# AlessioSam/LADiff

Measured on AMD Instinct MI355X. Metric: motions/sec (196-frame, 50-step DDIM, bs128), higher is better.
Workload: dtype f16x3+f32; 1 GPU; headline:ddim50_cfg7.5_b128_f196_c263_humanml3d; prompts_per_gpu=128, global_batch=128, frames=196, scheduler=ddim, denoising_steps=50, parallelism=dp1, loop=persistent pipeline kernel (16-row blocks x 86)

## Files before the change

include/ladiff_hip_debug.h:

```cpp
#ifndef LADIFF_HIP_DEBUG_H
#define LADIFF_HIP_DEBUG_H

#include "ladiff_hip.h"

#ifdef __cplusplus
extern "C" {
#endif

LADIFF_API int ladiff_debug_set_stage_waves(int waves_per_simd);
LADIFF_API int ladiff_debug_set_handoff(int tagged);
LADIFF_API int ladiff_debug_set_stage_plan(int v);
LADIFF_API int ladiff_debug_set_poll_pause(int mask, int len);
LADIFF_API int ladiff_debug_set_stage_delay(int mask, int len);
LADIFF_API int ladiff_debug_set_pacing(int eighths, int mask);
LADIFF_API int ladiff_debug_set_xcd_local(int on);
LADIFF_API int ladiff_debug_set_decoder_fusion(int on);
LADIFF_API int ladiff_debug_set_mlp_variant(int v);

LADIFF_API int ladiff_debug_set_loop_thresholds(int look_ahead_from, int small_upto);
LADIFF_API int ladiff_debug_set_graph_epoch_rule(int on);
LADIFF_API int ladiff_debug_graph_instantiations(void);

#ifdef LADIFF_STAMPS
LADIFF_API void ladiff_debug_set_stamps(unsigned long long* p);
LADIFF_API void ladiff_debug_set_sys_stamps(unsigned long long* p);
LADIFF_API void ladiff_debug_set_probe(int v);
#endif

#ifdef __cplusplus
}
#endif
#endif
```

ladiff_amd/_lib.py:

```python
import ctypes
import os
from ctypes import c_char_p, c_float, c_int, c_size_t, c_uint64, c_void_p

import numpy as np
import torch

_HERE = os.path.dirname(os.path.abspath(__file__))
LIB_PATH = os.path.join(_HERE, "libladiff_hip.so")

MAX_LATENTS = 8
MAX_FRAMES = 224
COEF_STRIDE = 8
ACT = {"none": 0, "relu": 1, "gelu": 2, "silu": 3, "qgelu": 4, "lrelu": 5}


class LadiffHipError(RuntimeError):
    pass


SPLIT_MODES = ("f16x3", "bf16x3", "split")


def is_split(precision):
    if precision == "fp32":
# ... 61 lines not shown
    "ladiff_debug_set_stage_plan": (c_int, [c_int]),
    "ladiff_debug_set_poll_pause": (c_int, [c_int, c_int]),
    "ladiff_debug_set_stage_delay": (c_int, [c_int, c_int]),
    "ladiff_debug_set_pacing": (c_int, [c_int, c_int]),
    "ladiff_debug_set_loop_thresholds": (c_int, [c_int, c_int]),
    "ladiff_debug_set_graph_epoch_rule": (c_int, [c_int]),
    "ladiff_debug_graph_instantiations": (c_int, []),
    "ladiff_sampler_set_fault": (c_int, [c_void_p, c_int, c_int]),
    "ladiff_sampler_set_noise_generator": (c_int, [c_void_p, c_uint64, ctypes.c_uint32, c_int]),
    "ladiff_noise_fill": (c_int, [c_uint64, ctypes.c_uint32, c_int, c_int, c_int, c_int, c_void_p, c_void_p]),
    "ladiff_reverse_workspace_bytes": (c_size_t, [c_int, c_int, c_int, c_int]),
    "ladiff_diffusion_reverse": (c_int, [c_void_p, c_void_p, c_void_p, c_uint64, c_void_p, c_void_p, c_void_p, c_void_p, c_void_p,
                                         c_void_p, c_void_p, c_void_p, c_float, c_float, c_int, c_int, c_int, c_int, c_int,
                                         c_void_p, c_void_p, c_size_t, c_int, c_void_p]),
    "ladiff_encoder_num_params": (c_int, []),
    "ladiff_encoder_param_name": (c_char_p, [c_int]),
    "ladiff_encoder_workspace_bytes": (c_size_t, [c_int, c_int, c_int, c_int]),
    "ladiff_vae_encode": (c_int, [c_void_p, c_void_p, c_void_p, c_void_p, c_void_p, c_void_p, c_int, c_int, c_int, c_int,
                                  c_void_p, c_void_p, c_void_p, c_void_p, c_size_t, c_void_p]),
    "ladiff_clip_num_params": (c_int, []),
    "ladiff_clip_param_name": (c_char_p, [c_int]),
    "ladiff_clip_workspace_bytes": (c_size_t, [c_int, c_int]),
    "ladiff_clip_text_encode": (c_int, [c_void_p, c_void_p, c_int, c_int, c_void_p, c_int, c_int, c_int, c_void_p, c_void_p,
                                        c_size_t, c_void_p]),
    "ladiff_clip_workspace_bytes_ragged": (c_size_t, [c_int, c_int]),
    "ladiff_clip_text_encode_ragged": (c_int, [c_void_p, c_void_p, c_int, c_int, c_void_p, c_int, c_int, c_int, c_void_p, c_void_p,
                                               c_void_p, c_int, c_void_p, c_void_p, c_size_t, c_void_p]),
    "ladiff_t2m_movement_num_params": (c_int, []),
    "ladiff_t2m_movement_param_name": (c_char_p, [c_int]),
    "ladiff_t2m_motion_num_params": (c_int, []),
    "ladiff_t2m_motion_param_name": (c_char_p, [c_int]),
    "ladiff_t2m_text_num_params": (c_int, []),
    "ladiff_t2m_text_param_name": (c_char_p, [c_int]),
    "ladiff_t2m_movement_workspace_bytes": (c_size_t, [c_int, c_int, c_int]),
    "ladiff_t2m_motion_workspace_bytes": (c_size_t, [c_int, c_int]),
    "ladiff_t2m_text_workspace_bytes": (c_size_t, [c_int, c_int]),
    "ladiff_t2m_movement_encode": (c_int, [c_void_p, c_void_p, c_int, c_int, c_int, c_int, c_void_p, c_void_p, c_size_t,
                                           c_void_p]),
    "ladiff_t2m_motion_encode": (c_int, [c_void_p, c_void_p, c_void_p, c_int, c_int, c_void_p, c_void_p, c_size_t, c_void_p]),
    "ladiff_t2m_text_encode": (c_int, [c_void_p, c_void_p, c_void_p, c_void_p, c_int, c_int, c_void_p, c_void_p, c_size_t,
                                       c_void_p]),
    "ladiff_feats2joints": (c_int, [c_void_p, c_void_p, c_void_p, c_int, c_int, c_int, c_int, c_void_p, c_void_p]),
    "ladiff_joint_ape_ave": (c_int, [c_void_p, c_void_p, c_void_p, c_void_p, c_int, c_int, c_int, c_void_p, c_float, c_void_p, c_void_p,
                                     c_void_p]),
    "ladiff_joint_mr": (c_int, [c_void_p, c_void_p, c_void_p, c_int, c_int, c_int, c_void_p, c_void_p, c_void_p]),
    "ladiff_decoder_workspace_bytes": (c_size_t, [c_int, c_int, c_int, c_int]),
    "ladiff_vae_decode": (c_int, [c_void_p, c_void_p, c_void_p, c_void_p, c_void_p, c_int, c_int, c_int, c_int, c_void_p,
                                  c_void_p, c_size_t, c_void_p]),
    "ladiff_debug_set_stage_waves": (c_int, [c_int]),
    "ladiff_debug_set_handoff": (c_int, [c_int]),
    "ladiff_debug_set_xcd_local": (c_int, [c_int]),
    "ladiff_debug_set_decoder_fusion": (c_int, [c_int]),
    "ladiff_debug_set_mlp_variant": (c_int, [c_int]),
    "ladiff_reverse_plan": (c_int, [c_int, c_int, c_void_p, c_int, c_int, c_int, c_int, c_void_p, c_void_p]),
    "ladiff_decoder_graph_create": (c_int, [ctypes.POINTER(c_void_p)]),
    "ladiff_decoder_graph_destroy": (c_int, [c_void_p]),
    "ladiff_vae_decode_graphed": (c_int, [c_void_p, c_void_p, c_void_p, c_uint64, c_void_p, c_void_p, c_void_p, c_void_p, c_int, c_int, c_int,
                                          c_int, c_int, c_void_p, c_void_p, c_size_t, c_void_p]),
    "ladiff_vae_decode_ragged": (c_int, [c_void_p, c_void_p, c_void_p, c_void_p, c_void_p, c_void_p, c_int, c_int, c_int, c_int,
                                         c_int, c_void_p, c_void_p, c_size_t, c_void_p]),
}

EXPORTS = tuple(_SIGNATURES)
_lib = None
LIB_PATH_BF16 = os.path.join(_HERE, "libladiff_hip_bf16.so")


def select_split_format(fmt):
    global LIB_PATH, _lib
    if fmt not in ("fp16", "bf16"):
        raise ValueError(f'split format must be "fp16" or "bf16", got {fmt!r}')
    path = LIB_PATH_BF16 if fmt == "bf16" else os.path.join(_HERE, "libladiff_hip.so")
    if _lib is not None and path != LIB_PATH:
        raise LadiffHipError("select_split_format() after the library has been used: weight tables of the other format exist")
    LIB_PATH = path


def lib():
    global _lib
    if _lib is None:
        if not os.path.exists(LIB_PATH):
            raise LadiffHipError(f"{LIB_PATH} not found: build it with `python -m ladiff_amd.build` "
                                 "(the HIP library is the only implementation of this path; there is no CPU fallback)")
        cdll = ctypes.CDLL(LIB_PATH)
        for name, (res, args) in _SIGNATURES.items():
            fn = getattr(cdll, name)
            fn.restype, fn.argtypes = res, args
        _lib = cdll
    return _lib


def check(rc):
    if rc != 0:
        raise LadiffHipError(f"libladiff_hip: {lib().ladiff_error_string(rc).decode()} (code {rc})")


def ptr(t, dtype=torch.float32):
    if t is None:
        return None
    if not t.is_cuda:
        raise LadiffHipError("libladiff_hip works on GPU tensors only; got a CPU tensor (no CPU fallback exists)")
    if t.dtype != dtype:
        raise LadiffHipError(f"expected {dtype}, got {t.dtype}")
    if not t.is_contiguous():
        raise LadiffHipError("expected a contiguous tensor")
    return t.data_ptr()
# ... 135 lines not shown
```

ladiff_amd/csrc/api.hip:

```cpp
#include <algorithm>
#include <cstdlib>
#include <cstring>
#include <vector>

#include "model.h"
#include "sampler.h"
#include "../../include/ladiff_hip_debug.h"

using namespace ladiff;

namespace {

inline hipStream_t S(ladiff_stream_t s) { return reinterpret_cast<hipStream_t>(s); }

bool all_set(const float* const* w, size_t n) {
    if (w == nullptr) return false;
    for (size_t i = 0; i < n; ++i)
        if (w[i] == nullptr) return false;
    return true;
}
template <class W>
bool load_weights(W& dst, const float* const* ptrs) {
    if (!all_set(ptrs, sizeof(W) / sizeof(const float*))) return false;
    std::memcpy(&dst, ptrs, sizeof(W));
// ... 194 lines not shown
    Sampler* sp = reinterpret_cast<Sampler*>(sampler);
    if (sp == nullptr) return 0;
    (void)hipDeviceSynchronize();
    sp->drain_retired();
    if (sp->exec) (void)hipGraphExecDestroy(sp->exec);
    if (sp->setup) (void)hipGraphExecDestroy(sp->setup);
    if (sp->ev0) (void)hipEventDestroy(sp->ev0);
    if (sp->ev1) (void)hipEventDestroy(sp->ev1);
    for (hipEvent_t e : sp->wev) (void)hipEventDestroy(e);
    sp->cap.destroy();
    delete sp;
    return 0;
}

int ladiff_reverse_plan(int B, int T, const int32_t* h_counts, int masked, int loop_mode, int f16x3, int cfg, int* rows_per_block, int* n_blocks) {
    LADIFF_CHECK_ARG(B >= 1 && T >= 1 && T <= LADIFF_MAX_LATENTS && loop_mode >= 1 && loop_mode <= 3 && rows_per_block && n_blocks);
    if (!cfg && masked && h_counts == nullptr) return LADIFF_ERR_UNSUPPORTED;
    std::vector<unsigned char> plan;
    int mr = 2, nb = 0;
    choose_plan(B, T, h_counts, masked != 0, loop_mode, f16x3 != 0, plan, &mr, &nb, cfg != 0);
    *rows_per_block = 16 * mr; *n_blocks = nb;
    return 0;
}

int ladiff_debug_set_stage_waves(int waves_per_simd) {
    LADIFF_CHECK_ARG(waves_per_simd == 1 || waves_per_simd == 2);
    g_waves16 = waves_per_simd;
    return 0;
}

int ladiff_debug_set_handoff(int tagged) {
    LADIFF_CHECK_ARG(tagged == 0 || tagged == 1);
    g_handoff = tagged;
    return 0;
}

int ladiff_debug_set_mlp_variant(int v) {
#ifdef LADIFF_STAMPS
    LADIFF_CHECK_ARG((v >= 0 && v <= 3) || (v >= 11 && v <= 17) || (v >= 21 && v <= 26));
#else
    LADIFF_CHECK_ARG(v >= 0 && v <= 3);
#endif
    g_mlp_variant = v;
    return 0;
}

int ladiff_debug_set_decoder_fusion(int on) {
    LADIFF_CHECK_ARG(on >= 0 && on <= 126 && (on & 3) != 3 && (on & 48) != 48);
    g_dec_out_cross = (on & 64) ? 0 : 1;
    g_dec_fused_mlp = on & 3;
    g_dec_small_rows_path = (on & 4) ? 0 : 1;
    g_dec_final_split = (on & 8) ? 0 : 1;
    g_dec_fused_attn = (on & 16) ? 0 : (on & 32) ? 2 : 1;
    return 0;
}

int ladiff_debug_set_stage_plan(int v) {
    LADIFF_CHECK_ARG(v >= 0 && v <= 1);
    g_stage_plan = v;
    return 0;
}

int ladiff_debug_set_poll_pause(int mask, int len) {
    LADIFF_CHECK_ARG(mask >= 0 && mask <= 255 && len >= 0 && len <= 64);
    g_poll_pause = mask | (len << 8);
    return 0;
}

int ladiff_debug_set_pacing(int eighths, int mask) {
    if (eighths == -1) { g_pace = -1; return 0; }
    LADIFF_CHECK_ARG(eighths >= 0 && eighths <= 8 && mask >= 0 && mask <= 255);
    g_pace = eighths | (mask << 8);
    return 0;
}

int ladiff_debug_set_stage_delay(int mask, int len) {
    LADIFF_CHECK_ARG(mask >= -1 && mask <= 255 && len >= 0 && len <= 64);
    g_stage_delay = mask < 0 ? -1 : (mask | (len << 8));
    return 0;
}

int ladiff_debug_set_loop_thresholds(int look_ahead_from, int small_upto) {
    LADIFF_CHECK_ARG(look_ahead_from >= -1 && small_upto >= -1);
    g_look_ahead_from = look_ahead_from;
    g_small_upto = small_upto;
    return 0;
}

int ladiff_debug_set_graph_epoch_rule(int on) {
    LADIFF_CHECK_ARG(on == 0 || on == 1);
    g_graph_epoch_rule = on;
    return 0;
}

int ladiff_debug_graph_instantiations(void) { return g_graph_instantiations.load(); }

int ladiff_debug_set_xcd_local(int on) {
    LADIFF_CHECK_ARG(on >= 0 && on <= 2);
    g_xcd_local = on;
    return 0;
}

int ladiff_sampler_set_loop(void* sampler, int mode) {
    Sampler* sp = reinterpret_cast<Sampler*>(sampler);
    LADIFF_CHECK_ARG(sp != nullptr && mode >= 0 && mode <= 3);
    sp->loop = mode != 0;
// ... 328 lines not shown
```

ladiff_amd/csrc/denoiser.hip:

```cpp
#include "model.h"

namespace ladiff {

static std::vector<std::string> block_prefixes(const char* root) {
    std::vector<std::string> v;
    for (int i = 0; i < NSKIP; ++i) v.push_back(std::string(root) + ".input_blocks." + std::to_string(i));
    v.push_back(std::string(root) + ".middle_block");
    for (int i = 0; i < NSKIP; ++i) v.push_back(std::string(root) + ".output_blocks." + std::to_string(i));
    return v;
}
static void wb(std::vector<std::string>& v, const std::string& p) { v.push_back(p + ".weight"); v.push_back(p + ".bias"); }
static void mha_names(std::vector<std::string>& v, const std::string& p) {
    v.push_back(p + ".in_proj_weight"); v.push_back(p + ".in_proj_bias"); wb(v, p + ".out_proj");
}
static void styl_names(std::vector<std::string>& v, const std::string& p) {
    wb(v, p + ".emb_layers.1"); wb(v, p + ".norm"); wb(v, p + ".out_layers.2");
}

const std::vector<std::string>& denoiser_param_names() {
    static const std::vector<std::string> names = [] {
        std::vector<std::string> v;
        wb(v, "time_embedding.linear_1"); wb(v, "time_embedding.linear_2"); wb(v, "emb_proj.1");
        v.push_back("query_pos.pe"); v.push_back("mem_pos.pe");
        wb(v, "encoder.norm");
// ... 63 lines not shown
        const DenLayerW& L = w.layer[l];
        float* base = tables + (size_t)l * DEN_LAYER_STRIDE;
        LADIFF_TRY(launch_gemm(lin(semb, D, L.ca_proj.emb, base + DEN_OFF_CA_MOD, DEN_STEP_STRIDE, n, 2 * D, D), s));
        LADIFF_TRY(launch_gemm(lin(semb, D, L.ffn_proj.emb, base + DEN_OFF_FFN_MOD, DEN_STEP_STRIDE, n, 2 * D, D), s));
        LinearW kvw{L.sa_attn.in_w + (size_t)D * D, L.sa_attn.in_b + D};
        LADIFF_TRY(launch_gemm(lin(temb, D, kvw, base + DEN_OFF_TIME_KV, DEN_STEP_STRIDE, n, 2 * D, D), s));
    }
    return 0;
}

static int denoiser_text_cache_general(const DenoiserW& w, const float* text, int B2, int N, float* cache, float* ws, size_t ws_floats,
                                       hipStream_t s) {
    const int R = B2 * N;
    const DenTextWs t = den_text_layout(ws, B2, 1, N);
    if (ws_floats < t.total) return LADIFF_ERR_WORKSPACE;
    const DenTextCache c = den_text_cache_layout(cache, B2, 1, N);
    float *rl = t.rl, *tn = t.tn, *key = t.key, *val = t.val, *tproj = c.tproj, *tkv = c.tkv, *catt = c.catt;
    LADIFF_TRY(launch_relu(text, rl, (size_t)R * TEXT_DIM, s));
    LADIFF_TRY(launch_gemm(lin(rl, TEXT_DIM, w.emb_proj, tproj, D, R, D, TEXT_DIM), s));
    for (int l = 0; l < NL; ++l) {
        const DenLayerW& L = w.layer[l];
        LinearW kvw{L.sa_attn.in_w + (size_t)D * D, L.sa_attn.in_b + D};
        LADIFF_TRY(launch_gemm(lin(tproj, D, kvw, tkv + (size_t)l * R * 2 * D, 2 * D, R, 2 * D, D), s));
        LADIFF_TRY(launch_layernorm(tproj, L.ca_text_norm.g, L.ca_text_norm.b, tn, R, s));
        LADIFF_TRY(launch_gemm(lin(tn, D, L.ca_key, key, D, R, D, D), s));
        LADIFF_TRY(launch_gemm(lin(tn, D, L.ca_value, val, D, R, D, D), s));
        LADIFF_TRY(launch_lca_kv(key, val, B2, N, catt + (size_t)l * B2 * H * DH * DH, s));
    }
    return 0;
}

int denoiser_text_static(const DenoiserW& w, const float* text, int B2, float* cache, float* ws, size_t ws_floats, hipStream_t s) {
    const DenTextWs t = den_text_layout(ws, B2, 0, 1);
    if (ws_floats < t.total) return LADIFF_ERR_WORKSPACE;
    const DenTextCache c = den_text_cache_layout(cache, B2, 0, 1);
    float *rl = t.rl, *tn = t.tn, *tproj = c.tproj, *tkv = c.tkv, *nval = c.nval;
    LADIFF_TRY(launch_relu(text, rl, (size_t)B2 * TEXT_DIM, s));
    LADIFF_TRY(launch_gemm(lin(rl, TEXT_DIM, w.emb_proj, tproj, D, B2, D, TEXT_DIM), s));
    GemmArgs kv[NL], val[NL];
    RowBatch ln;
    for (int l = 0; l < NL; ++l) {
        const DenLayerW& L = w.layer[l];
        LinearW kvw{L.sa_attn.in_w + (size_t)D * D, L.sa_attn.in_b + D};
        kv[l] = lin(tproj, D, kvw, tkv + (size_t)l * B2 * 2 * D, 2 * D, B2, 2 * D, D);
        ln.a[l] = tproj; ln.g[l] = L.ca_text_norm.g; ln.b[l] = L.ca_text_norm.b; ln.y[l] = tn + (size_t)l * B2 * D;
        val[l] = lin(tn + (size_t)l * B2 * D, D, L.ca_value, nval + (size_t)l * B2 * D, D, B2, D, D);
        val[l].ln_g = L.ca_proj.norm.g; val[l].ln_b = L.ca_proj.norm.b;
    }
    LADIFF_TRY(launch_gemm_batch(kv, NL, s));
    LADIFF_TRY(launch_layernorm_batch(ln, NL, B2, s));
    return launch_gemm_batch(val, NL, s);
}

int denoiser_ctab(const DenoiserW& w, const float* tables_lo, int n, float* cache, int B2, float* u, size_t u_floats, hipStream_t s,
                  const DenoiserW* wsp) {
    const int R = B2 + 1;
    const size_t u_all = den_text_layout(nullptr, B2, n, 1).u_floats;
    if (u_floats < u_all / NL) return LADIFF_ERR_WORKSPACE;
    const DenTextCache c = den_text_cache_layout(cache, B2, n, 1);
    const float* nval = c.nval;
    float* ctab = c.ctab;
    if (u_floats >= u_all) {
        RowBatch rb;
        GemmArgs g[NL];
        for (int l = 0; l < NL; ++l) {
            const DenLayerW& L = w.layer[l];
            float* ul = u + (size_t)l * n * R * D;
            rb.a[l] = nval + (size_t)l * B2 * D; rb.g[l] = L.ca_proj.norm.b;
            rb.b[l] = tables_lo + (size_t)l * DEN_LAYER_STRIDE + DEN_OFF_CA_MOD; rb.y[l] = ul;
            g[l] = lin(ul, D, L.ca_proj.out, ctab + (size_t)l * n * R * D, D, n * R, D, D);
            if (wsp != nullptr) { g[l].W = wsp->layer[l].ca_proj.out.w; g[l].split = 1; }
        }
        LADIFF_TRY(launch_ca_table_input_batch(rb, NL, DEN_STEP_STRIDE, n, B2, s, wsp != nullptr ? 1 : 0));
        return launch_gemm_batch(g, NL, s);
    }
    for (int l = 0; l < NL; ++l) {
        const DenLayerW& L = w.layer[l];
        LADIFF_TRY(launch_ca_table_input(nval + (size_t)l * B2 * D, L.ca_proj.norm.b, tables_lo + (size_t)l * DEN_LAYER_STRIDE + DEN_OFF_CA_MOD,
                                         DEN_STEP_STRIDE, n, B2, u, s));
        LADIFF_TRY(launch_gemm(lin(u, D, L.ca_proj.out, ctab + (size_t)l * n * R * D, D, n * R, D, D), s));
    }
    return 0;
}

int denoiser_text_cache(const DenoiserW& w, const float* text, int B2, const float* tables, int n, float* cache,
                        float* ws, size_t ws_floats, hipStream_t s, int ntxt) {
    if (ntxt > 1) return denoiser_text_cache_general(w, text, B2, ntxt, cache, ws, ws_floats, s);
    const DenTextWs t = den_text_layout(ws, B2, n, 1);
    if (ws_floats < t.total) return LADIFF_ERR_WORKSPACE;
    LADIFF_TRY(denoiser_text_static(w, text, B2, cache, ws, ws_floats, s));
    return denoiser_ctab(w, tables, n, cache, B2, t.u, t.u_floats, s, nullptr);
}

int linear_cross_attention(const DenoiserW& w, int layer, const float* x, const float* xf, const float* emb, const int32_t* counts,
                           int B, int T, int N, float* out, float* ws, size_t ws_floats, hipStream_t s) {
    if (layer < 0 || layer >= NL || T < 1 || T > LADIFF_MAX_LATENTS || N < 1) return LADIFF_ERR_SHAPE;
    const LcaWs a = lca_layout(ws, B, T, N);
    if (ws_floats < a.total) return LADIFF_ERR_WORKSPACE;
    const DenLayerW& L = w.layer[layer];
    const int R = B * N, M = B * T;
    float *tn = a.tn, *key = a.key, *val = a.val, *catt = a.catt, *xn = a.xn, *q = a.q, *semb = a.semb, *mod = a.mod;
    LADIFF_TRY(launch_layernorm(xf, L.ca_text_norm.g, L.ca_text_norm.b, tn, R, s));
    LADIFF_TRY(launch_gemm(lin(tn, D, L.ca_key, key, D, R, D, D), s));
    LADIFF_TRY(launch_gemm(lin(tn, D, L.ca_value, val, D, R, D, D), s));
    LADIFF_TRY(launch_lca_kv(key, val, B, N, catt, s));
    LADIFF_TRY(launch_layernorm(x, L.ca_norm.g, L.ca_norm.b, xn, M, s));
    LADIFF_TRY(launch_gemm(lin(xn, D, L.ca_query, q, D, M, D, D), s));
    LADIFF_TRY(launch_silu(emb, semb, (size_t)B * D, s));
    LADIFF_TRY(launch_gemm(lin(semb, D, L.ca_proj.emb, mod, 2 * D, B, 2 * D, D), s));
    LADIFF_TRY(launch_lca_apply(q, catt, counts, B, 0, B, T, mod, 0, 2 * D, nullptr, L.ca_proj.norm.g, L.ca_proj.norm.b, xn, s));
    GemmArgs g = lin(xn, D, L.ca_proj.out, out, D, M, D, D);
    g.res = x; g.ldres = D;
    return launch_gemm(g, s);
}
// ... 133 lines not shown
```

ladiff_amd/csrc/gemm.h:

```cpp
#pragma once
#include "common.h"

namespace ladiff {

struct GemmArgs {
    const float* A = nullptr;  int lda = 0;
    const float* A2 = nullptr; int lda2 = 0;
    int K1 = 0;
    const float* W = nullptr;  int ldw = 0;
    const float* bias = nullptr;
    float* Y = nullptr;        int ldy = 0;
    float* Ys = nullptr;
    int split = 0;
    int M = 0, N = 0, K = 0;
    int act = ACT_NONE;
    const float* res = nullptr; int ldres = 0;
    const float* ln_g = nullptr; const float* ln_b = nullptr;
    const float* ln2_g = nullptr; const float* ln2_b = nullptr;
    const float* mod = nullptr;
    const int32_t* d_step = nullptr; int mod_stride = 0;
    int post_act = ACT_NONE;
    const int32_t* row_len = nullptr; int rows_per_item = 0;
    const int32_t* row_map = nullptr;
    int ksplit = 1; size_t plane = 0;
};

int launch_gemm(const GemmArgs& a, hipStream_t stream);
constexpr int GEMM_BATCH_MAX = 9;
struct GemmBatch { GemmArgs a[GEMM_BATCH_MAX]; };
int launch_gemm_batch(const GemmArgs* list, int n, hipStream_t stream);
int launch_gemm_big_batch(const GemmBatch& b, int n, hipStream_t stream);
bool gemm_big_supported(const GemmArgs& a);
int launch_gemm_big(const GemmArgs& a, hipStream_t stream);

}
```

ladiff_amd/csrc/gemm_big.hip:

```cpp
#include "gemm.h"

namespace ladiff {

namespace {
constexpr int BKB = 32;
template <int N> __device__ __forceinline__ void wait_vm() { asm volatile("s_waitcnt vmcnt(%0)" ::"n"(N) : "memory"); }
__device__ __forceinline__ void dma16(const float* g, float* l) {
    __builtin_amdgcn_global_load_lds(g, (__attribute__((address_space(3))) void*)l, 16, 0, 0);
}
}

template <int BM, int BN, int WM, int WN, bool LN>
__device__ __forceinline__ void gemm_big_body(const GemmArgs& p) {
    constexpr int NW = 4;
    static_assert(WM * WN == NW, "four waves");
    constexpr int TMW = BM / WM, TNW = BN / WN, RM = TMW / 32, RN = TNW / 32;
    constexpr int ROWS = BM + BN;
    constexpr int STAGE = ROWS * BKB;
    constexpr int GRP = 8 * NW;
    constexpr int GA = BM / GRP, GT = ROWS / GRP;
    static_assert(BM % GRP == 0 && BN % GRP == 0, "tiles are multiples of 32 rows");
    constexpr int CLD = BN + 4;
    constexpr int LDSF = (2 * STAGE > BM * CLD) ? 2 * STAGE : BM * CLD;
    constexpr int LPR = BN / 4;
    constexpr int RPI = 64 / LPR;
    constexpr int EI = BM / NW / RPI;
    static_assert(!LN || BN == 256, "LayerNorm needs whole rows");

    __shared__ __attribute__((aligned(1024))) float lds[LDSF];

    const int tid = threadIdx.x, lane = tid & 63;
    const int wave = __builtin_amdgcn_readfirstlane(tid >> 6);
    const int wm = wave / WN, wn = wave % WN;
    const int nbn = p.N / BN;
    const int nbm = (p.M + BM - 1) / BM;
    const int xcd = blockIdx.x & 7, local = blockIdx.x >> 3;
    const int bm = (local / nbn) * 8 + xcd, bn = local % nbn;
    if (bm >= nbm) return;
    const int row0 = bm * BM, col0 = bn * BN;
    const int nk = p.K / BKB;

    const int rl = 8 * wave + (lane >> 3);
    const int kl = (((lane & 7) ^ ((rl >> 1) & 7)) << 2);
    float* const lbase = lds + 8 * wave * BKB;
    auto issue = [&](int kt, int buf) __attribute__((always_inline)) {
        const int k0 = kt * BKB;
        const float* abase; int ald;
        if (k0 < p.K1) { abase = p.A + k0; ald = p.lda; } else { abase = p.A2 + (k0 - p.K1); ald = p.lda2; }
#pragma unroll
        for (int g = 0; g < GT; ++g) {
            const float* src;
            if (g < GA) {
                int gr = row0 + GRP * g + rl; gr = gr < p.M ? gr : p.M - 1;
// ... 54 lines not shown
                if (gr < p.M) rv[e] = ld4(p.res + (size_t)gr * p.ldres + col0 + ec);
            }
        }
        compute(buf);
    }
    __builtin_amdgcn_s_barrier();

    float* ct = lds;
#pragma unroll
    for (int i = 0; i < RM; ++i)
#pragma unroll
        for (int j = 0; j < RN; ++j)
#pragma unroll
            for (int r = 0; r < 16; ++r)
                ct[(wm * TMW + i * 32 + (r & 3) + 8 * (r >> 2) + 4 * (lane >> 5)) * CLD + wn * TNW + j * 32 + (lane & 31)] = acc[i][j][r];
    asm volatile("s_waitcnt vmcnt(0) lgkmcnt(0)" ::: "memory");
    __builtin_amdgcn_s_barrier();
#pragma unroll
    for (int e = 0; e < EI; ++e) reg_touch(rv[e]);

    f32x4 bv = {0.f, 0.f, 0.f, 0.f};
    if (p.bias != nullptr) bv = ld4(p.bias + col0 + ec);
    f32x4 g1 = bv, b1 = bv, g2 = bv, b2 = bv;
    if constexpr (LN) {
        g1 = ld4(p.ln_g + ec); b1 = ld4(p.ln_b + ec);
        if (p.ln2_g != nullptr) { g2 = ld4(p.ln2_g + ec); b2 = ld4(p.ln2_b + ec); }
    }
    act_dispatch(p.act, [&](auto ACT) __attribute__((always_inline)) {
#pragma unroll
    for (int e = 0; e < EI; ++e) {
        const int lr = er + e * RPI;
        const int gr = row0 + lr;
        f32x4 v = ld4(ct + lr * CLD + ec);
#pragma unroll
        for (int q = 0; q < 4; ++q) v[q] = act_c<decltype(ACT)::value>(v[q] + bv[q]) + rv[e][q];
        if constexpr (LN) {
#pragma unroll
            for (int pass = 0; pass < 2; ++pass) {
                if (pass == 1 && p.ln2_g == nullptr) break;
                const float mean = wave_sum((v[0] + v[1]) + (v[2] + v[3])) * (1.f / 256.f);
                float sq = 0.f;
#pragma unroll
                for (int q = 0; q < 4; ++q) { const float d = v[q] - mean; sq += d * d; }
                const float rstd = rsqrtf(wave_sum(sq) * (1.f / 256.f) + LN_EPS);
#pragma unroll
                for (int q = 0; q < 4; ++q) v[q] = (v[q] - mean) * rstd * (pass ? g2[q] : g1[q]) + (pass ? b2[q] : b1[q]);
            }
        }
        if (gr < p.M) st4(p.Y + (size_t)gr * p.ldy + col0 + ec, v);
    }
    });
}

template <int BM, int BN>
__device__ __forceinline__ void gemm_big_split_body(const GemmArgs& p) {
    constexpr int NW = 4, WM = 2, WN = 2;
    constexpr int TMW = BM / WM, TNW = BN / WN, RM = TMW / 16, RN = TNW / 16;
    constexpr int ROWS = BM + BN;
    constexpr int STAGE = ROWS * 32;
    constexpr int GRP = 8 * NW;
    constexpr int GA = BM / GRP, GT = ROWS / GRP;
    constexpr int CLD = BN + 4;
    constexpr int LPR = BN / 4, RPI = 64 / LPR, EI = BM / NW / RPI;
    constexpr int LDSF = (2 * STAGE > BM * CLD) ? 2 * STAGE : BM * CLD;

    __shared__ __attribute__((aligned(1024))) float lds[LDSF];

    const int tid = threadIdx.x, lane = tid & 63;
    const int wave = __builtin_amdgcn_readfirstlane(tid >> 6);
    const int wm = wave / WN, wn = wave % WN;
    const int argM = pin_s(p.M), argK1 = pin_s(p.K1), ldy = pin_s(p.ldy), act = pin_s(p.act);
    float* const argY = pin_s(p.Y); float* const argYs = pin_s(p.Ys);
    const int nbn = p.N / BN;
    const int nbm = (argM + BM - 1) / BM;
    const int xcd = blockIdx.x & 7, local = blockIdx.x >> 3;
    const int bm = (local / nbn) * 8 + xcd, bn = local % nbn;
    if (bm >= nbm) return;
    const int row0 = bm * BM, col0 = bn * BN;
    const int ksplit = pin_s(p.ksplit), kz = ksplit > 1 ? (int)blockIdx.y : 0;
    const int nk_all = p.K / 32, nk = nk_all / ksplit, kt0 = kz * nk;

    const int rl = 8 * wave + (lane >> 3);
    const int cs = (lane & 7) ^ ((rl >> 1) & 7);
    const int kl = (cs < 4 ? cs * 4 : 32 + (cs - 4) * 4);
    float* const lbase = lds + 8 * wave * 32;
    auto issue = [&](int ktl, int buf) __attribute__((always_inline)) {
        const int kt = kt0 + ktl;
        const int k0 = (kt >> 1) * 64, hf = (kt & 1) * 16;
        const float* abase; int ald;
        if (k0 < argK1) { abase = p.A + k0; ald = p.lda; } else { abase = p.A2 + (k0 - argK1); ald = p.lda2; }
#pragma unroll
        for (int g = 0; g < GT; ++g) {
            const float* src;
            if (g < GA) {
                int gr = row0 + GRP * g + rl; gr = gr < argM ? gr : argM - 1;
                src = abase + (size_t)gr * ald + hf + kl;
            } else {
                src = p.W + (size_t)(col0 + GRP * (g - GA) + rl) * p.ldw + k0 + hf + kl;
            }
            dma16(src, lbase + buf * STAGE + GRP * g * 32);
        }
    };

    f32x4 acc[RM][RN];
#pragma unroll
    for (int i = 0; i < RM; ++i)
#pragma unroll
        for (int j = 0; j < RN; ++j) acc[i][j] = f32x4{0.f, 0.f, 0.f, 0.f};

    const int frow = lane & 15, fk = lane >> 4;
    const int sw = (frow >> 1) & 7;
    auto compute = [&](int buf) __attribute__((always_inline)) {
        const float* sa = lds + buf * STAGE + (wm * TMW) * 32;
        const float* sb = lds + buf * STAGE + (BM + wn * TNW) * 32;
        s16x8 ah[RM], al[RM], bh[RN], bl[RN];
#pragma unroll
        for (int i = 0; i < RM; ++i) {
            const int r = i * 16 + frow;
            ah[i] = __builtin_bit_cast(s16x8, ld4(sa + r * 32 + ((fk ^ sw) << 2)));
            al[i] = __builtin_bit_cast(s16x8, ld4(sa + r * 32 + (((4 + fk) ^ sw) << 2)));
        }
#pragma unroll
        for (int j = 0; j < RN; ++j) {
            const int r = j * 16 + frow;
            bh[j] = __builtin_bit_cast(s16x8, ld4(sb + r * 32 + ((fk ^ sw) << 2)));
            bl[j] = __builtin_bit_cast(s16x8, ld4(sb + r * 32 + (((4 + fk) ^ sw) << 2)));
        }
#pragma unroll
        for (int i = 0; i < RM; ++i)
#pragma unroll
            for (int j = 0; j < RN; ++j) acc[i][j] = MFMA16_S16(al[i], bh[j], acc[i][j], 0, 0, 0);
#pragma unroll
        for (int i = 0; i < RM; ++i)
#pragma unroll
            for (int j = 0; j < RN; ++j) acc[i][j] = MFMA16_S16(ah[i], bl[j], acc[i][j], 0, 0, 0);
#pragma unroll
        for (int i = 0; i < RM; ++i)
#pragma unroll
            for (int j = 0; j < RN; ++j) acc[i][j] = MFMA16_S16(ah[i], bh[j], acc[i][j], 0, 0, 0);
    };

    const int er = wave * (BM / NW) + lane / LPR;
    const int ec = 4 * (lane % LPR);
    f32x4 rv[EI];
#pragma unroll
    for (int e = 0; e < EI; ++e) rv[e] = f32x4{0.f, 0.f, 0.f, 0.f};
    f32x4 bv = {0.f, 0.f, 0.f, 0.f};

    issue(0, 0);
    for (int kt = 0; kt < nk; ++kt) {
        const int buf = kt & 1;
        wait_vm<0>();
        __builtin_amdgcn_s_barrier();
        if (kt + 1 < nk) issue(kt + 1, buf ^ 1);
        if (kt == nk - 1 && ksplit == 1) {
            if (p.bias != nullptr) bv = ld4(p.bias + col0 + ec);
            if (p.res != nullptr) {
#pragma unroll
                for (int e = 0; e < EI; ++e) {
                    const int gr = row0 + er + e * RPI;
                    if (gr < argM) rv[e] = ld4(p.res + (size_t)gr * p.ldres + col0 + ec);
                }
            }
        }
        compute(buf);
    }
    __builtin_amdgcn_s_barrier();

    float* ct = lds;
#pragma unroll
    for (int i = 0; i < RM; ++i)
#pragma unroll
        for (int j = 0; j < RN; ++j)
#pragma unroll
            for (int r = 0; r < 4; ++r)
                ct[(wm * TMW + i * 16 + 4 * (lane >> 4) + r) * CLD + wn * TNW + j * 16 + (lane & 15)] = acc[i][j][r];
    asm volatile("s_waitcnt vmcnt(0) lgkmcnt(0)" ::: "memory");
    __builtin_amdgcn_s_barrier();
    reg_touch(bv);
#pragma unroll
    for (int e = 0; e < EI; ++e) reg_touch(rv[e]);

    if (ksplit > 1) {
        float* const Yz = argY + (size_t)kz * p.plane;
#pragma unroll
        for (int e = 0; e < EI; ++e) {
            const int lr = er + e * RPI;
            const int gr = row0 + lr;
            if (gr < argM) st4g(Yz + (size_t)gr * ldy + col0 + ec, ld4(ct + lr * CLD + ec));
        }
        return;
    }
    act_dispatch(act, [&](auto ACT) __attribute__((always_inline)) {
#pragma unroll
        for (int e = 0; e < EI; ++e) {
            const int lr = er + e * RPI;
            const int gr = row0 + lr;
            f32x4 v = ld4(ct + lr * CLD + ec);
#pragma unroll
            for (int q = 0; q < 4; ++q) v[q] = act_c<decltype(ACT)::value>(v[q] + bv[q]) + rv[e][q];
            if (gr < argM) {
                if (argY != nullptr) st4g(argY + (size_t)gr * ldy + col0 + ec, v);
                if (argYs != nullptr) store_split4g(argYs + (size_t)gr * ldy, col0 + ec, v);
            }
        }
    });
}

template <int BM, int BN>
__global__ __launch_bounds__(256, 2) void gemm_big_split_kernel(const GemmArgs p) { gemm_big_split_body<BM, BN>(p); }
template <int BM, int BN>
__global__ __launch_bounds__(256, 2) void gemm_big_split_batch_kernel(const GemmBatch b) { gemm_big_split_body<BM, BN>(b.a[blockIdx.y]); }

template <int BM, int BN, int WM, int WN, bool LN>
__global__ __launch_bounds__(256) void gemm_big_kernel(const GemmArgs p) { gemm_big_body<BM, BN, WM, WN, LN>(p); }
template <int BM, int BN, int WM, int WN, bool LN>
__global__ __launch_bounds__(256) void gemm_big_batch_kernel(const GemmBatch b) { gemm_big_body<BM, BN, WM, WN, LN>(b.a[blockIdx.y]); }

template <int BM, int BN, int WM, int WN, bool LN>
static int launch_big_batch(const GemmBatch& b, int n, hipStream_t s) {
    const GemmArgs& a = b.a[0];
    const int nbm = (a.M + BM - 1) / BM, nbn = a.N / BN;
    const int grid = ((nbm + 7) / 8) * 8 * nbn;
    hipLaunchKernelGGL((gemm_big_batch_kernel<BM, BN, WM, WN, LN>), dim3(grid, n), dim3(256), 0, s, b);
    LADIFF_LAUNCH_CHECK();
    return 0;
}

template <int BM, int BN, int WM, int WN, bool LN>
static int launch_big(const GemmArgs& a, hipStream_t s) {
    const int nbm = (a.M + BM - 1) / BM, nbn = a.N / BN;
    const int grid = ((nbm + 7) / 8) * 8 * nbn;
    hipLaunchKernelGGL((gemm_big_kernel<BM, BN, WM, WN, LN>), dim3(grid), dim3(256), 0, s, a);
    LADIFF_LAUNCH_CHECK();
    return 0;
}

bool gemm_big_supported(const GemmArgs& a) {
    if (a.split) return a.M > 0 && a.K % 64 == 0 && a.K1 % 64 == 0 && a.N % 128 == 0 && a.lda % 4 == 0 && a.ldw % 4 == 0 && (!a.A2 || a.lda2 % 4 == 0) &&
                        a.ldy % 64 == 0 && !a.ln_g && !a.mod && !a.row_len && !a.row_map && a.post_act == ACT_NONE && (a.Y || a.Ys);
    if (a.M < 4096 || a.K % BKB || a.K1 % BKB || (a.lda % 4) || (a.ldw % 4) || (a.A2 && (a.lda2 % 4))) return false;
    if ((a.ldy % 4) || (a.res && (a.ldres % 4)) || a.mod || a.row_len || a.row_map || a.post_act != ACT_NONE) return false;
    if (a.ln_g != nullptr) return a.N == 256;
    return a.N % 128 == 0;
}

int launch_gemm_big(const GemmArgs& a, hipStream_t s) {
    if (a.split) {
        const int nbm = (a.M + 127) / 128, nbn = a.N / 128;
        const int ks = a.ksplit > 1 ? a.ksplit : 1;
        if (ks > 1 && ((a.K / 32) % ks != 0 || a.Y == nullptr || a.Ys != nullptr || a.plane == 0)) return LADIFF_ERR_ARG;
        if (nbm * nbn <= 256 && a.M > 64) {
            const int nbm64 = (a.M + 63) / 64;
            hipLaunchKernelGGL((gemm_big_split_kernel<64, 128>), dim3(((nbm64 + 7) / 8) * 8 * nbn, ks), dim3(256), 0, s, a);
        } else {
            hipLaunchKernelGGL((gemm_big_split_kernel<128, 128>), dim3(((nbm + 7) / 8) * 8 * nbn, ks), dim3(256), 0, s, a);
        }
        LADIFF_LAUNCH_CHECK();
        return 0;
    }
    if (a.ksplit > 1) return LADIFF_ERR_ARG;
    if (a.ln_g != nullptr) return launch_big<64, 256, 2, 2, true>(a, s);
    return launch_big<128, 128, 2, 2, false>(a, s);
}

int launch_gemm_big_batch(const GemmBatch& b, int n, hipStream_t s) {
    for (int i = 0; i < n; ++i) if (b.a[i].ksplit > 1) return LADIFF_ERR_ARG;
    if (b.a[0].split) {
        const GemmArgs& a = b.a[0];
        const int nbm = (a.M + 127) / 128, nbn = a.N / 128;
        hipLaunchKernelGGL((gemm_big_split_batch_kernel<128, 128>), dim3(((nbm + 7) / 8) * 8 * nbn, n), dim3(256), 0, s, b);
        LADIFF_LAUNCH_CHECK();
        return 0;
    }
    if (b.a[0].ln_g != nullptr) return launch_big_batch<64, 256, 2, 2, true>(b, n, s);
    return launch_big_batch<128, 128, 2, 2, false>(b, n, s);
}

}
```

ladiff_amd/csrc/kernels.h:

```cpp
#pragma once
#include "common.h"
#include "noise_gen.h"

namespace ladiff {

enum RedMode : int { RED_PLAIN = 0, RED_LN = 1, RED_LN_ADD = 2, RED_LN_MOD = 3 };
int launch_reduce_rows(const float* P, int S, int M, const float* bias, const float* res, int mode, const float* g,
                       const float* b, const float* tab, int tab_step_stride, const int32_t* d_step,
                       const int32_t* counts, int Bs, int T, int pad_row, int b_off, float* out, float* outs, hipStream_t s,
                       const int32_t* d_base = nullptr, const float* g2 = nullptr, const float* b2 = nullptr);
int launch_split_rows(const float* x, float* y, int R, int K, hipStream_t s);
int launch_gather_rows(const float* src, const int32_t* index, int n_rows, int row_floats, float* dst, hipStream_t s);
int launch_split_range_stats(const float* const* xs, const int64_t* counts, int n, int64_t max_count, unsigned long long* stats,
                             hipStream_t s);
int launch_layernorm(const float* x, const float* g, const float* b, float* y, int M, hipStream_t s);
constexpr int DEC_PREP_MAX = 9;
struct DecCrossPrepBatch { const float* kv[DEC_PREP_MAX]; const float* wq[DEC_PREP_MAX]; const float* bq[DEC_PREP_MAX];
                           const float* wo[DEC_PREP_MAX]; float* gu[DEC_PREP_MAX]; };
constexpr int ROW_BATCH_MAX = 9;
struct RowBatch { const float* a[ROW_BATCH_MAX]; const float* g[ROW_BATCH_MAX]; const float* b[ROW_BATCH_MAX]; float* y[ROW_BATCH_MAX]; };
int launch_layernorm_batch(const RowBatch& rb, int n, int M, hipStream_t s);
int launch_ca_table_input_batch(const RowBatch& rb, int n_layers, int step_stride, int n, int B2, hipStream_t s, int split_out = 0);
int launch_ca_table_input(const float* nval, const float* beta, const float* mod, int step_stride, int n, int B2, float* u,
                          hipStream_t s);
int launch_add_pe(const float* sample, const float* pe, int Bs, int b_off, int b_n, int T, float* x, float* xs, hipStream_t s);
int launch_broadcast_pe(const float* pe, int B, int F, float* x, float* xs, hipStream_t s);
int launch_broadcast_pe_ragged(const float* pe, const int32_t* row_off, int B, int F, int F_out, float* x, float* xs, int32_t* row_out,
                               hipStream_t s);
int launch_relu(const float* x, float* y, size_t n, hipStream_t s);
int launch_pad_rows(const float* src, const float* srcb, float* dst, float* dstb, int C, int Np, hipStream_t s);
int launch_zero_fill(float* x, size_t n, hipStream_t s);
int launch_silu(const float* x, float* y, size_t n, hipStream_t s);
int launch_sinusoid(const int64_t* t, int n, float* out, hipStream_t s);
int launch_cfg_step(const float* eps, float* lat, const float* coef, const int32_t* d_step, const float* noise,
                    float g, int cfg, int B, int T, hipStream_t s);
int launch_advance(int32_t* d_step, hipStream_t s);
int launch_step_tail(float* x, float* xs, const float* ng, const float* nb, float* lat, const float* coef, int32_t* d_step,
                     const float* noise, const float* pe, float g, int cfg, int B, int T, hipStream_t s, const NoiseGen& gen = NoiseGen{0u, 0u, 0u, 0});
int launch_noise_fill(const NoiseGen& gen, int step0, int n, int B, int T, float* out, hipStream_t s);
int launch_init_latents(const float* noise, const int32_t* counts, float sigma, float* lat, int B, int T, hipStream_t s);
int launch_finalize_latents(const float* lat, const int32_t* counts, float* z, int B, int T, hipStream_t s, const unsigned* status = nullptr);

int launch_dec_qkv_attn(const float* xs, const float* w, const float* bias, const int32_t* lengths, const int32_t* row_off, float* out,
                        int B, int F, int split_out, hipStream_t s);
int launch_scatter_feats(const float* tmp, int ldt, int C, int M, int F, const int32_t* row_len, const int32_t* row_map, float* feats,
                         hipStream_t s);
int launch_pad_cols(const float* x, float* y, int R, int C, int Cp, hipStream_t s);
int launch_encoder_assemble(const float* token, const float* emb, const float* pe, const int32_t* lengths,
                            const int32_t* counts, int B, int F, int T, float* x, float* xs, uint32_t* keybits, hipStream_t s);
int launch_encoder_finalize(const float* out, const float* eps, const int32_t* counts, int B, int T, int S, float* mu, float* sd,
                            float* latent, hipStream_t s);

int launch_lca_kv(const float* key, const float* value, int B, int N, float* att, hipStream_t s);
int launch_lca_apply(const float* q, const float* att, const int32_t* counts, int Bs, int b_off, int b_n, int T, const float* mod,
                     int step_stride, int sample_stride, const int32_t* d_step, const float* g, const float* be, float* u,
                     hipStream_t s);
int launch_denoiser_self_attention_general(const float* qkv, const float* text_kv, int N, const float* tables, int kv_off,
                                           int step_stride, const int32_t* d_step, const int32_t* counts, int Bs, int b_off,
                                           int b_n, int T, float* out, hipStream_t s);

int launch_decoder_cross_prep(const DecCrossPrepBatch& pb, int n, int B, int T, hipStream_t s);
int launch_decoder_out_cross(const float* att_s, const float* x0, const float* wo_s, const float* bo, const float* g1, const float* b1,
                             const float* bo_c, const float* g2, const float* b2, const int32_t* counts, int B, int F, int T,
                             const float* gu_ws, float* y, float* ys, hipStream_t s, const int32_t* row_off);
int launch_decoder_cross_apply(const float* x, const float* bo, const float* g2, const float* b2, const int32_t* counts, int B, int F,
                               int T, const float* gu_ws, float* y, float* ys, hipStream_t s, const int32_t* row_off = nullptr,
                               const float* g1 = nullptr, const float* b1 = nullptr);

int launch_feats2joints(const float* feats, const float* mean, const float* stdv, int B, int F, int C, int J, float* joints,
                        hipStream_t s);

int launch_joint_ape_ave(const float* rst, const float* ref, const int32_t* lengths, int B, int F, int J, const int32_t* part_idx,
                         float factor, float* seq_rows, double* acc, hipStream_t s);
int launch_joint_mr(const float* rst, const float* ref, int B, int F, int J, float* seq_rows, double* acc, hipStream_t s);

int launch_denoiser_self_attention(const float* qkv, const float* text_kv, const float* tables, int kv_off,
                                   int step_stride, const int32_t* d_step, const int32_t* counts, int Bs, int b_off,
// ... 12 lines not shown
```

ladiff_amd/csrc/model.h:

```cpp
#pragma once
#include <atomic>
#include "gemm.h"
#include "gemm_kr.h"
#include "graph_key.h"
#include "kernels.h"
#include "systolic_plan.h"
#include "weights.h"
#include "workspace.h"

namespace ladiff {

int denoiser_time_tables(const DenoiserW& w, const float* sinus, int n, float* tables, float* ws, size_t ws_floats, hipStream_t s);
int denoiser_text_cache(const DenoiserW& w, const float* text, int B2, const float* tables, int n_steps, float* cache,
                        float* ws, size_t ws_floats, hipStream_t s, int ntxt = 1);
int denoiser_forward(const DenoiserW& w, const DenoiserW* w_split, const float* tables, const int32_t* d_step,
                     const float* cache, int n_steps, const float* sample, int Bs, int dup, int T, const int32_t* counts, float* eps, float* ws,
                     size_t ws_floats, hipStream_t s, int b_lo = 0, int b_n = -1, int loop_mode = 0, int ntxt = 1,
                     const int32_t* d_base = nullptr);
int denoiser_text_static(const DenoiserW& w, const float* text, int B2, float* cache, float* ws, size_t ws_floats, hipStream_t s);
int denoiser_ctab(const DenoiserW& w, const float* tables_lo, int n, float* cache, int B2, float* u, size_t u_floats, hipStream_t s,
                  const DenoiserW* w_split = nullptr);
int linear_cross_attention(const DenoiserW& w, int layer, const float* x, const float* xf, const float* emb, const int32_t* counts,
                           int B, int T, int N, float* out, float* ws, size_t ws_floats, hipStream_t s);

struct Sampler;
int diffusion_reverse(Sampler* sp, const DenoiserW& w, const DenoiserW* w_split, const ReverseArgs& a);

extern std::atomic<int> g_dec_fused_mlp;
extern std::atomic<int> g_dec_small_rows_path;
extern std::atomic<int> g_dec_final_split;
extern std::atomic<int> g_dec_out_cross;
extern std::atomic<int> g_stage_plan;
extern std::atomic<int> g_poll_pause;
extern std::atomic<int> g_stage_delay;
extern std::atomic<int> g_pace;
extern std::atomic<int> g_look_ahead_from, g_small_upto;
extern std::atomic<int> g_dec_fused_attn;
extern std::atomic<int> g_mlp_variant;
int dec_mlp_prepare();
int dec_qkv_attn_prepare();
int dec_cross_prepare();
int dec_mlp_min_rows();
int vae_decode(const DecoderW& w, const DecoderW* w_split, const float* z, const int32_t* lengths, const int32_t* counts,
               const int32_t* row_off, int R, int B, int F, int T, int C, float* feats, float* ws, size_t ws_floats, hipStream_t s);

int launch_dec_mlp(const float* xs, const float* x, const float* w1, const float* b1, const float* w2, const float* b2, const float* g3,
                   const float* be3, const float* g4, const float* be4, float* y, float* ys, int M, hipStream_t s);

int vae_encode(const EncoderW& w, const EncoderW* w_split, const float* features, const int32_t* lengths,
               const int32_t* counts, const float* eps, int B, int F, int T, int C, float* mu, float* sd, float* latent, float* ws,
               size_t ws_floats, hipStream_t s);

#ifdef LADIFF_STAMPS
extern unsigned long long* g_sys_stamps;
extern int g_sys_probe;
#endif
bool sys_supported(int B, int T, int cfg, bool split);
extern std::atomic<int> g_waves16;
extern std::atomic<int> g_handoff;
int sys_reset_status(float* ws, hipStream_t s);
extern std::atomic<int> g_xcd_local;
int sys_build_stages(const DenoiserW& W, const DenoiserW& WS, float* ws, int MR, int NB, std::vector<unsigned char>& host);
int launch_systolic_loop(const DenoiserW& W, float* ws, const float* tables, const float* tkv, const float* ctab, int n_ctab,
                         const float* coef, const float* noise, float* lat, const int32_t* counts, float gscale, int B, int T,
                         int step_lo, int n, int fp32, int MR, int NB, hipStream_t s, int cfg = 1, int fault_wg = -1,
                         unsigned long long timeout_ticks = 0, const NoiseGen& gen = NoiseGen{0u, 0u, 0u, 0});

int launch_qkv_attention(const float* x, const float* w, const float* bias, const float* text_kv, const float* tables,
                         int kv_off, int step_stride, const int32_t* d_step, const int32_t* counts, int Bs, int b_off,
                         int b_n, int T, float* out, hipStream_t s);

int clip_text_encode(const ClipW& w, const ClipW* w_split, int n_layers, int vocab, const int64_t* ids, int B, int S, int L,
                     float* out, float* ws, size_t ws_floats, hipStream_t s, const int32_t* seq_len = nullptr,
                     const int32_t* row_off = nullptr, const int32_t* row_seq = nullptr, int total_rows = 0);

const std::vector<std::string>& t2m_move_param_names();
const std::vector<std::string>& t2m_motion_param_names();
const std::vector<std::string>& t2m_text_param_names();
int t2m_movement_encode(const float* const* w, const float* feats, int ld, int B, int F, int Cin, float* out, float* ws,
                        size_t ws_floats, hipStream_t s);
int t2m_motion_encode(const float* const* w, const float* mov, const int32_t* m_lens, int B, int T, float* out, float* ws,
                      size_t ws_floats, hipStream_t s);
int t2m_text_encode(const float* const* w, const float* word_embs, const float* pos_onehot, const int32_t* cap_lens, int B, int L,
                    float* out, float* ws, size_t ws_floats, hipStream_t s);

}
```

Measured before the change: 11410 motions/s.

## Fuse cross-attention table input generation into the split GEMM loader

```diff
diff --git a/include/ladiff_hip_debug.h b/include/ladiff_hip_debug.h
--- a/include/ladiff_hip_debug.h
+++ b/include/ladiff_hip_debug.h
@@ -15,6 +15,7 @@
 LADIFF_API int ladiff_debug_set_pacing(int eighths, int mask);
 LADIFF_API int ladiff_debug_set_xcd_local(int on);
 LADIFF_API int ladiff_debug_set_decoder_fusion(int on);
+LADIFF_API int ladiff_debug_set_ctab_fusion(int on);
 LADIFF_API int ladiff_debug_set_mlp_variant(int v);
 
 LADIFF_API int ladiff_debug_set_loop_thresholds(int look_ahead_from, int small_upto);
diff --git a/ladiff_amd/_lib.py b/ladiff_amd/_lib.py
--- a/ladiff_amd/_lib.py
+++ b/ladiff_amd/_lib.py
@@ -137,6 +137,7 @@
     "ladiff_debug_set_xcd_local": (c_int, [c_int]),
     "ladiff_debug_set_decoder_fusion": (c_int, [c_int]),
     "ladiff_debug_set_mlp_variant": (c_int, [c_int]),
+    "ladiff_debug_set_ctab_fusion": (c_int, [c_int]),
     "ladiff_reverse_plan": (c_int, [c_int, c_int, c_void_p, c_int, c_int, c_int, c_int, c_void_p, c_void_p]),
     "ladiff_decoder_graph_create": (c_int, [ctypes.POINTER(c_void_p)]),
     "ladiff_decoder_graph_destroy": (c_int, [c_void_p]),
diff --git a/ladiff_amd/csrc/api.hip b/ladiff_amd/csrc/api.hip
--- a/ladiff_amd/csrc/api.hip
+++ b/ladiff_amd/csrc/api.hip
@@ -270,6 +270,12 @@
     g_dec_small_rows_path = (on & 4) ? 0 : 1;
     g_dec_final_split = (on & 8) ? 0 : 1;
     g_dec_fused_attn = (on & 16) ? 0 : (on & 32) ? 2 : 1;
+    return 0;
+}
+
+int ladiff_debug_set_ctab_fusion(int on) {
+    LADIFF_CHECK_ARG(on == 0 || on == 1);
+    g_ctab_fused = on;
     return 0;
 }
 
diff --git a/ladiff_amd/csrc/denoiser.hip b/ladiff_amd/csrc/denoiser.hip
--- a/ladiff_amd/csrc/denoiser.hip
+++ b/ladiff_amd/csrc/denoiser.hip
@@ -139,6 +139,8 @@
     return launch_gemm_batch(val, NL, s);
 }
 
+std::atomic<int> g_ctab_fused{1};
+
 int denoiser_ctab(const DenoiserW& w, const float* tables_lo, int n, float* cache, int B2, float* u, size_t u_floats, hipStream_t s,
                   const DenoiserW* wsp) {
     const int R = B2 + 1;
@@ -147,6 +149,18 @@
     const DenTextCache c = den_text_cache_layout(cache, B2, n, 1);
     const float* nval = c.nval;
     float* ctab = c.ctab;
+    if (u_floats >= u_all && wsp != nullptr && g_ctab_fused.load()) {
+        CtabBatch cb;
+        for (int l = 0; l < NL; ++l) {
+            const DenLayerW& L = w.layer[l];
+            cb.a[l] = lin(nullptr, D, L.ca_proj.out, ctab + (size_t)l * n * R * D, D, n * R, D, D);
+            cb.a[l].W = wsp->layer[l].ca_proj.out.w; cb.a[l].split = 1; cb.a[l].K1 = D;
+            cb.rows[l].nval = nval + (size_t)l * B2 * D; cb.rows[l].beta = L.ca_proj.norm.b;
+            cb.rows[l].mod = tables_lo + (size_t)l * DEN_LAYER_STRIDE + DEN_OFF_CA_MOD;
+            cb.rows[l].step_stride = DEN_STEP_STRIDE; cb.rows[l].B2 = B2;
+        }
+        return launch_ctab_fused(cb, NL, s);
+    }
     if (u_floats >= u_all) {
         RowBatch rb;
         GemmArgs g[NL];
diff --git a/ladiff_amd/csrc/gemm.h b/ladiff_amd/csrc/gemm.h
--- a/ladiff_amd/csrc/gemm.h
+++ b/ladiff_amd/csrc/gemm.h
@@ -30,6 +30,8 @@
 struct GemmBatch { GemmArgs a[GEMM_BATCH_MAX]; };
 int launch_gemm_batch(const GemmArgs* list, int n, hipStream_t stream);
 int launch_gemm_big_batch(const GemmBatch& b, int n, hipStream_t stream);
+struct CtabRows { const float* nval = nullptr; const float* beta = nullptr; const float* mod = nullptr; int step_stride = 0, B2 = 0; };
+struct CtabBatch { GemmArgs a[GEMM_BATCH_MAX]; CtabRows rows[GEMM_BATCH_MAX]; };
 bool gemm_big_supported(const GemmArgs& a);
 int launch_gemm_big(const GemmArgs& a, hipStream_t stream);
 
diff --git a/ladiff_amd/csrc/gemm_big.hip b/ladiff_amd/csrc/gemm_big.hip
--- a/ladiff_amd/csrc/gemm_big.hip
+++ b/ladiff_amd/csrc/gemm_big.hip
@@ -1,4 +1,5 @@
 #include "gemm.h"
+#include "kernels.h"
 
 namespace ladiff {
 
@@ -159,9 +160,9 @@
     });
 }
 
-template <int BM, int BN>
-__device__ __forceinline__ void gemm_big_split_body(const GemmArgs& p) {
-    constexpr int NW = 4, WM = 2, WN = 2;
+template <int BM, int BN, bool GEN = false>
+__device__ __forceinline__ void gemm_big_split_body(const GemmArgs& p, const CtabRows* cg = nullptr) {
+    constexpr int NW = 4, WM = BN >= 256 ? 1 : 2, WN = NW / WM;
     constexpr int TMW = BM / WM, TNW = BN / WN, RM = TMW / 16, RN = TNW / 16;
     constexpr int ROWS = BM + BN;
     constexpr int STAGE = ROWS * 32;
@@ -194,10 +195,12 @@
     auto issue = [&](int ktl, int buf) __attribute__((always_inline)) {
         const int kt = kt0 + ktl;
         const int k0 = (kt >> 1) * 64, hf = (kt & 1) * 16;
-        const float* abase; int ald;
-        if (k0 < argK1) { abase = p.A + k0; ald = p.lda; } else { abase = p.A2 + (k0 - argK1); ald = p.lda2; }
-#pragma unroll
-        for (int g = 0; g < GT; ++g) {
+        const float* abase = nullptr; int ald = 0;
+        if constexpr (!GEN) {
+            if (k0 < argK1) { abase = p.A + k0; ald = p.lda; } else { abase = p.A2 + (k0 - argK1); ald = p.lda2; }
+        }
+#pragma unroll
+        for (int g = GEN ? GA : 0; g < GT; ++g) {
             const float* src;
             if (g < GA) {
                 int gr = row0 + GRP * g + rl; gr = gr < argM ? gr : argM - 1;
@@ -209,6 +212,56 @@
         }
     };
 
+    constexpr int GP = GEN ? BM / 64 : 1;
+    const float* vrow[GP]; const float* mrow[GP];
+    int lhi[GP], llo[GP];
+    f32x4 gin[GP][6];
+    if constexpr (GEN) {
+        static_assert(BM % 64 == 0, "whole passes");
+        const int R = cg->B2 + 1, o = lane & 3;
+#pragma unroll
+        for (int q = 0; q < GP; ++q) {
+            const int r = 64 * q + 16 * wave + (lane >> 2);
+            int gr = row0 + r; gr = gr < argM ? gr : argM - 1;
+            const int step = gr / R, b = gr - step * R;
+            vrow[q] = (b < cg->B2 ? cg->nval + (size_t)b * 256 : cg->beta) + 8 * o;
+            mrow[q] = cg->mod + (size_t)step * cg->step_stride + 8 * o;
+            const int sw = (r >> 1) & 7;
+            lhi[q] = r * 32 + ((o ^ sw) << 2); llo[q] = r * 32 + (((4 + o) ^ sw) << 2);
+        }
+    }
+    auto gen_load = [&](int kt) __attribute__((always_inline)) {
+        const int c = kt * 32;
+#pragma unroll
+        for (int q = 0; q < GP; ++q) {
+            gin[q][0] = ld4g(vrow[q] + c); gin[q][1] = ld4g(vrow[q] + c + 4);
+            gin[q][2] = ld4g(mrow[q] + c); gin[q][3] = ld4g(mrow[q] + c + 4);
+            gin[q][4] = ld4g(mrow[q] + 256 + c); gin[q][5] = ld4g(mrow[q] + 256 + c + 4);
+        }
+    };
+    auto gen_touch = [&]() __attribute__((always_inline)) {
+#pragma unroll
+        for (int q = 0; q < GP; ++q)
+#pragma unroll
+            for (int i = 0; i < 6; ++i) reg_touch(gin[q][i]);
+    };
+    auto gen_store = [&](int buf) __attribute__((always_inline)) {
+#pragma unroll
+        for (int q = 0; q < GP; ++q) {
+            f32x4 a, b;
+#pragma unroll
+            for (int i = 0; i < 4; ++i) {
+                a[i] = silu(gin[q][0][i] * (1.f + gin[q][2][i]) + gin[q][4][i]);
+                b[i] = silu(gin[q][1][i] * (1.f + gin[q][3][i]) + gin[q][5][i]);
+            }
+            s16x8 hi, lo;
+            split8(a, b, hi, lo);
+            *reinterpret_cast<s16x8*>(lds + buf * STAGE + lhi[q]) = hi;
+            *reinterpret_cast<s16x8*>(lds + buf * STAGE + llo[q]) = lo;
+        }
+    };
+    (void)gen_load; (void)gen_touch; (void)gen_store;
+
     f32x4 acc[RM][RN];
 #pragma unroll
     for (int i = 0; i < RM; ++i)
@@ -255,14 +308,30 @@
     f32x4 bv = {0.f, 0.f, 0.f, 0.f};
 
     issue(0, 0);
+    if constexpr (GEN) {
+        gen_load(0);
+        wait_vm<0>();
+        gen_touch();
+        gen_store(0);
+        if (nk > 1) gen_load(1);
+    }
     for (int kt = 0; kt < nk; ++kt) {
         const int buf = kt & 1;
-        wait_vm<0>();
+        if constexpr (GEN) {
+            asm volatile("s_waitcnt vmcnt(0) lgkmcnt(0)" ::: "memory");
+            gen_touch();
+        } else {
+            wait_vm<0>();
+        }
         __builtin_amdgcn_s_barrier();
         if (kt + 1 < nk) issue(kt + 1, buf ^ 1);
+        if constexpr (GEN) {
+            if (kt + 1 < nk) gen_store(buf ^ 1);
+            if (kt + 2 < nk) gen_load(kt + 2);
+        }
         if (kt == nk - 1 && ksplit == 1) {
             if (p.bias != nullptr) bv = ld4(p.bias + col0 + ec);
-            if (p.res != nullptr) {
+            if (!GEN && p.res != nullptr) {
 #pragma unroll
                 for (int e = 0; e < EI; ++e) {
                     const int gr = row0 + er + e * RPI;
@@ -285,8 +354,10 @@
     asm volatile("s_waitcnt vmcnt(0) lgkmcnt(0)" ::: "memory");
     __builtin_amdgcn_s_barrier();
     reg_touch(bv);
-#pragma unroll
-    for (int e = 0; e < EI; ++e) reg_touch(rv[e]);
+    if constexpr (!GEN) {
+#pragma unroll
+        for (int e = 0; e < EI; ++e) reg_touch(rv[e]);
+    }
 
     if (ksplit > 1) {
         float* const Yz = argY + (size_t)kz * p.plane;
@@ -318,6 +389,13 @@
 __global__ __launch_bounds__(256, 2) void gemm_big_split_kernel(const GemmArgs p) { gemm_big_split_body<BM, BN>(p); }
 template <int BM, int BN>
 __global__ __launch_bounds__(256, 2) void gemm_big_split_batch_kernel(const GemmBatch b) { gemm_big_split_body<BM, BN>(b.a[blockIdx.y]); }
+
+static_assert(sizeof(CtabBatch) <= 4096, "kernel arguments");
+template <int BM, int BN>
+__global__ __launch_bounds__(256, 2) void gemm_ctab_fused_kernel(const CtabBatch b) {
+    static_assert(BN == 256, "a row's values are computed once: the tile spans N");
+    gemm_big_split_body<BM, BN, true>(b.a[blockIdx.y], &b.rows[blockIdx.y]);
+}
 
 template <int BM, int BN, int WM, int WN, bool LN>
 __global__ __launch_bounds__(256) void gemm_big_kernel(const GemmArgs p) { gemm_big_body<BM, BN, WM, WN, LN>(p); }
@@ -384,4 +462,22 @@
     return launch_big_batch<128, 128, 2, 2, false>(b, n, s);
 }
 
-}
+int launch_ctab_fused(const CtabBatch& b, int n, hipStream_t s) {
+    LADIFF_CHECK_ARG(n >= 1 && n <= GEMM_BATCH_MAX);
+    const GemmArgs& a = b.a[0];
+    for (int i = 0; i < n; ++i) {
+        const GemmArgs& g = b.a[i];
+        const CtabRows& r = b.rows[i];
+        LADIFF_CHECK_ARG(g.split && g.W && g.Y && !g.Ys && !g.A2 && !g.res && !g.ln_g && !g.mod && !g.row_len && !g.row_map && g.ksplit <= 1 &&
+                         g.post_act == ACT_NONE);
+        LADIFF_CHECK_ARG(g.M == a.M && g.N == 256 && g.K == 256 && g.K1 == 256 && g.ldw % 4 == 0 && g.ldy % 64 == 0);
+        LADIFF_CHECK_ARG(r.nval && r.beta && r.mod && r.B2 >= 1 && r.step_stride >= 512 && g.M % (r.B2 + 1) == 0);
+    }
+    if (a.M == 0) return 0;
+    const int nbm = (a.M + 63) / 64;
+    hipLaunchKernelGGL((gemm_ctab_fused_kernel<64, 256>), dim3(((nbm + 7) / 8) * 8, n), dim3(256), 0, s, b);
+    LADIFF_LAUNCH_CHECK();
+    return 0;
+}
+
+}
diff --git a/ladiff_amd/csrc/kernels.h b/ladiff_amd/csrc/kernels.h
--- a/ladiff_amd/csrc/kernels.h
+++ b/ladiff_amd/csrc/kernels.h
@@ -1,5 +1,6 @@
 #pragma once
 #include "common.h"
+#include "gemm.h"
 #include "noise_gen.h"
 
 namespace ladiff {
@@ -23,6 +24,7 @@
 int launch_ca_table_input_batch(const RowBatch& rb, int n_layers, int step_stride, int n, int B2, hipStream_t s, int split_out = 0);
 int launch_ca_table_input(const float* nval, const float* beta, const float* mod, int step_stride, int n, int B2, float* u,
                           hipStream_t s);
+int launch_ctab_fused(const CtabBatch& b, int n_layers, hipStream_t s);
 int launch_add_pe(const float* sample, const float* pe, int Bs, int b_off, int b_n, int T, float* x, float* xs, hipStream_t s);
 int launch_broadcast_pe(const float* pe, int B, int F, float* x, float* xs, hipStream_t s);
 int launch_broadcast_pe_ragged(const float* pe, const int32_t* row_off, int B, int F, int F_out, float* x, float* xs, int32_t* row_out,
diff --git a/ladiff_amd/csrc/model.h b/ladiff_amd/csrc/model.h
--- a/ladiff_amd/csrc/model.h
+++ b/ladiff_amd/csrc/model.h
@@ -37,6 +37,7 @@
 extern std::atomic<int> g_look_ahead_from, g_small_upto;
 extern std::atomic<int> g_dec_fused_attn;
 extern std::atomic<int> g_mlp_variant;
+extern std::atomic<int> g_ctab_fused;
 int dec_mlp_prepare();
 int dec_qkv_attn_prepare();
 int dec_cross_prepare();
```

After: 11470 motions/s (median of 6 runs). Within noise of the previous version (+0.5%).
